# oraclefina/MSPI

Hardware: AMD Instinct MI355X
Metric: clips_per_sec (higher is better)
Workload: dtype f32 storage/accumulate; GEMMs as f16x3 split products on the f16 MFMA pipe; 1 GPU; x3dl motion encoder + ConvNeXt-T + ResNet18 audio + SyncBlock + decoder (AudioVisualSaliencyModel forward), batch 8/GPU, clips 3x16x224x224, spectrogram 1x257x300, inputs resident in HBM; global_batch=8, launch=hipGraph replay (mspi_amd.runtime.GraphPipeline), 2 batches in flight, stream_layout=2, parallelism=single GPU

## Files before the change

### include/mspi_hip.h

```cpp
#ifndef MSPI_HIP_H
#define MSPI_HIP_H

#include <stddef.h>
#include <stdint.h>

#ifdef __cplusplus
extern "C" {
#endif

#define MSPI_ABI_VERSION 2

typedef void* mspi_stream_t;

enum {
  MSPI_OK = 0,
  MSPI_EINVAL = -1,
  MSPI_ELAUNCH = -2,
  MSPI_ENODEV = -3
};

enum { MSPI_ACT_NONE = 0, MSPI_ACT_RELU = 1, MSPI_ACT_GELU = 2, MSPI_ACT_SIGMOID = 3, MSPI_ACT_SWISH = 4 };

enum { MSPI_PREC_F32 = 0, MSPI_PREC_F16X3 = 1 };

// ... 18 lines not shown
  int32_t prec;
  float w_scale;
  int32_t tile;
  const void* w_blocked;
} MspiConvDesc;

int mspi_conv_fwd(const MspiConvDesc* d, const float* x, const float* w, const float* bias ,
                  const float* res , const float* gate ,
                  float* y, mspi_stream_t stream);

size_t mspi_conv_splitk_ws_bytes(const MspiConvDesc* d, int32_t ksplit);
int mspi_conv_splitk_fwd(const MspiConvDesc* d, const float* x, const float* w, const float* bias, const float* res,
                         float* y, void* workspace, int32_t ksplit, mspi_stream_t stream);
int mspi_conv_variant(const MspiConvDesc* d, const float* x, const float* gate, int32_t ksplit);

int mspi_conv_last_config(void);

typedef struct MspiDwConvDesc {
  int32_t N, T, H, W, C;
  int64_t ldx, ldy;
  int32_t kT, kH, kW;
  int32_t strT, strH, strW;
  int32_t padT, padH, padW;
  int32_t To, Ho, Wo;
  int32_t act;
} MspiDwConvDesc;

int mspi_dwconv_fwd(const MspiDwConvDesc* d, const float* x, const float* w, const float* bias,
                    float* y, float* pool , mspi_stream_t stream);
int mspi_dwconv_pool_rows(const MspiDwConvDesc* d);
// ... 50 lines not shown
  float wa_scale;
} MspiX3dAbDesc;

int mspi_x3d_ab_supported(const MspiX3dAbDesc* d);
int mspi_x3d_ab_pool_rows(const MspiX3dAbDesc* d);
size_t mspi_x3d_ab_packed_bytes(int32_t Cin, int32_t Cmid);
int mspi_x3d_ab_fwd(const MspiX3dAbDesc* d, const void* x, const void* wa_packed, const void* bias_a, const void* wb,
                    const void* bias_b, void* u, void* pool , mspi_stream_t stream);
int mspi_x3d_ab_variant(const MspiX3dAbDesc* d);

int mspi_maxpool_fwd(const MspiDwConvDesc* d, const float* x, float* y, mspi_stream_t stream);

int mspi_upsample_fwd(const float* src, int64_t lds, float* dst, int64_t ldd, int32_t NT, int32_t H,
                      int32_t W, int32_t C, int32_t factor, int32_t accumulate, int32_t act,
                      mspi_stream_t stream);

int mspi_space_to_depth(const float* x, int64_t ldx, float* y, int64_t ldy, int32_t NT, int32_t H, int32_t W,
                        int32_t C, mspi_stream_t stream);

int mspi_rowgate(float* x, int64_t ldx, const float* mask, int64_t M, int32_t C, mspi_stream_t stream);

int mspi_logsumexp_sub(float* x, int32_t N, int32_t L, mspi_stream_t stream);

int mspi_mean_rows(const float* x, int64_t ldx, int64_t rows_per_sample_stride, float* out, int32_t N,
                   int32_t R, int32_t C, mspi_stream_t stream);

int mspi_mean_rows_slices(int32_t R);
int mspi_mean_rows_ws(const float* x, int64_t ldx, int64_t rows_per_sample_stride, float* out, float* ws, int32_t N,
                      int32_t R, int32_t C, mspi_stream_t stream);

// ... 113 lines not shown
```

### mspi_amd/_lib.py

```python
import ctypes as C
import os

_HERE = os.path.dirname(os.path.abspath(__file__))
LIB_PATH = os.environ.get("MSPI_LIB_PATH") or os.path.join(_HERE, "csrc", "libmspi_hip.so")

ACT_NONE, ACT_RELU, ACT_GELU, ACT_SIGMOID, ACT_SWISH = range(5)
PREC_F32, PREC_F16X3 = 0, 1


class MspiError(RuntimeError):
    pass


class ConvDesc(C.Structure):
    _fields_ = [
        ("N", C.c_int32), ("T", C.c_int32), ("H", C.c_int32), ("W", C.c_int32), ("C", C.c_int32),
        ("sN", C.c_int64), ("sT", C.c_int64), ("sH", C.c_int64), ("sW", C.c_int64), ("sC", C.c_int64),
        ("kT", C.c_int32), ("kH", C.c_int32), ("kW", C.c_int32),
        ("strT", C.c_int32), ("strH", C.c_int32), ("strW", C.c_int32),
        ("padT", C.c_int32), ("padH", C.c_int32), ("padW", C.c_int32),
        ("To", C.c_int32), ("Ho", C.c_int32), ("Wo", C.c_int32),
        ("Cout", C.c_int32),
        ("ldy", C.c_int64), ("ldw", C.c_int64), ("ldr", C.c_int64),
        ("act", C.c_int32),
# ... 74 lines not shown
class PermuteDesc(C.Structure):
    _fields_ = [("dims", C.c_int32 * 6), ("strides", C.c_int64 * 6), ("src_elems", C.c_int64)]


_P = C.c_void_p
_SIGNATURES = {
    "mspi_version": (C.c_int, []),
    "mspi_last_error": (C.c_char_p, []),
    "mspi_device_count": (C.c_int, []),
    "mspi_set_status_word": (C.c_int, [_P]),
    "mspi_conv_last_config": (C.c_int, []),
    "mspi_conv_splitk_ws_bytes": (C.c_size_t, [C.POINTER(ConvDesc), C.c_int32]),
    "mspi_conv_splitk_fwd": (C.c_int, [C.POINTER(ConvDesc), _P, _P, _P, _P, _P, _P, C.c_int32, _P]),
    "mspi_conv_fwd": (C.c_int, [C.POINTER(ConvDesc), _P, _P, _P, _P, _P, _P, _P]),
    "mspi_conv_variant": (C.c_int, [C.POINTER(ConvDesc), _P, _P, C.c_int32]),
    "mspi_dwconv_fwd": (C.c_int, [C.POINTER(DwConvDesc), _P, _P, _P, _P, _P, _P]),
    "mspi_dwconv_pool_rows": (C.c_int, [C.POINTER(DwConvDesc)]),
    "mspi_dwconv_variant": (C.c_int, [C.POINTER(DwConvDesc)]),
    "mspi_se_gate": (C.c_int, [_P, C.c_int32, C.c_float, _P, _P, _P, _P, _P, C.c_int32, C.c_int32, C.c_int32, _P]),
    "mspi_se_gate_variant": (C.c_int, [C.c_int32, C.c_int32]),
    "mspi_layernorm_variant": (C.c_int, [C.c_int32, C.c_int32]),
    "mspi_layernorm_fwd": (C.c_int, [_P, C.c_int64, C.c_int64, _P, C.c_int64, C.c_int64, _P, _P, C.c_float, C.c_int32,
                                      C.c_int32, C.c_int32, C.c_int32, _P, _P]),
    "mspi_attn_fwd": (C.c_int, [C.POINTER(AttnDesc), _P, _P, _P, _P, _P, _P, _P, _P, _P]),
    "mspi_attn_ws_bytes": (C.c_size_t, [C.POINTER(AttnDesc)]),
    "mspi_attn_fwd_ws": (C.c_int, [C.POINTER(AttnDesc), _P, _P, _P, _P, _P, _P, _P, _P, _P, _P]),
    "mspi_attn_variant": (C.c_int, [C.POINTER(AttnDesc), C.c_int32, C.c_int32, C.c_int32, C.c_int32]),
    "mspi_space_to_depth": (C.c_int, [_P, C.c_int64, _P, C.c_int64, C.c_int32, C.c_int32, C.c_int32, C.c_int32, _P]),
    "mspi_mvit_qk_augment": (C.c_int, [C.POINTER(MvitAugDesc), _P, _P, _P, _P, _P, _P, _P, _P]),
    "mspi_mvit_qk_augment_p": (C.c_int, [C.POINTER(MvitAugDesc), _P, _P, _P, C.c_int64, _P, _P, _P, _P, _P, _P]),
    "mspi_maxpool_fwd": (C.c_int, [C.POINTER(DwConvDesc), _P, _P, _P]),
    "mspi_upsample_fwd": (C.c_int, [_P, C.c_int64, _P, C.c_int64, C.c_int32, C.c_int32, C.c_int32, C.c_int32,
                                     C.c_int32, C.c_int32, C.c_int32, _P]),
    "mspi_rowgate": (C.c_int, [_P, C.c_int64, _P, C.c_int64, C.c_int32, _P]),
    "mspi_logsumexp_sub": (C.c_int, [_P, C.c_int32, C.c_int32, _P]),
    "mspi_mean_rows": (C.c_int, [_P, C.c_int64, C.c_int64, _P, C.c_int32, C.c_int32, C.c_int32, _P]),
    "mspi_mean_rows_slices": (C.c_int, [C.c_int32]),
    "mspi_mean_rows_ws": (C.c_int, [_P, C.c_int64, C.c_int64, _P, _P, C.c_int32, C.c_int32, C.c_int32, _P]),
    "mspi_neg_cosine": (C.c_int, [_P, _P, _P, C.c_int32, C.c_int32, C.c_float, C.c_int32, _P]),
    "mspi_add": (C.c_int, [_P, _P, _P, C.c_int64, _P]),
    "mspi_permute_fwd": (C.c_int, [C.POINTER(PermuteDesc), _P, _P, _P]),
    "mspi_permute_variant": (C.c_int, [C.POINTER(PermuteDesc), _P, _P]),
    "mspi_gated_sum_fwd": (C.c_int, [_P, _P, _P, _P, _P, C.c_int32, C.c_int64, C.c_int32, C.c_int32, _P]),
    "mspi_logspec_fwd": (C.c_int, [_P, C.c_int64, _P, _P, C.c_int32, _P, _P, C.c_int32, _P]),
    "mspi_resize_norm_fwd": (C.c_int, [_P, C.c_int32, C.c_int32, _P, _P, C.c_int64, C.c_int32, C.c_int32, _P, _P, C.c_int32,
                                        _P, _P, C.c_int32, _P, _P, _P]),
    "mspi_clip_resize_plan": (C.c_int, [_P, C.c_int32, C.c_int32, C.c_int32, C.c_int32, C.c_int32, _P]),
    "mspi_clip_resize_norm_fwd": (C.c_int, [_P, C.c_int32, C.c_int32, C.c_int32, _P, _P, _P, C.c_int32, C.c_int32, C.c_int64,
# ... 65 lines not shown
```

### mspi_amd/csrc/rowops.hip

```cpp
#include "common.h"

namespace mspi {

constexpr int LN_MAXC = 3072;

template <int LPR, int VPT>
__global__ __launch_bounds__(256) void layernorm_kernel(const float* __restrict__ x, long ldx, long sNx,
                                                        float* __restrict__ y, long ldy, long sNy,
                                                        const float* __restrict__ gamma,
                                                        const float* __restrict__ beta, float eps, long M, int R, int C,
                                                        int act, const float* __restrict__ table,
                                                        _Float16* __restrict__ ys, long ldys, long yplane) {
  constexpr int RPW = 64 / LPR;
  const int lane = threadIdx.x & 63;
  const int sub = lane % LPR;
  const long row = ((long)blockIdx.x * 4 + (threadIdx.x >> 6)) * RPW + lane / LPR;
  const bool rok = row < M;
  const long rr = rok ? row : 0;
  const long n = (long)((unsigned)rr / (unsigned)R);
  const int r = (int)(rr - n * R);
  const int nv = C >> 2;
  const float* xr = x + n * sNx + (long)r * ldx;
  float4 v[VPT];
  float s = 0.f;
// ... 187 lines not shown
    if (accumulate) {
      const float4 p = *reinterpret_cast<const float4*>(d);
      o.x += p.x; o.y += p.y; o.z += p.z; o.w += p.w;
    }
    if (act != MSPI_ACT_NONE) {
      auto fin = [&](auto act_c) {
        constexpr int ACT = decltype(act_c)::value;
        o.x = act_apply(o.x, ACT); o.y = act_apply(o.y, ACT); o.z = act_apply(o.z, ACT); o.w = act_apply(o.w, ACT);
      };
      MSPI_DISPATCH_ACT(act, fin)
    }
    *reinterpret_cast<float4*>(d) = o;
  }
}

__global__ __launch_bounds__(256) void s2d_kernel(const float* __restrict__ x, long ldx, float* __restrict__ y, long ldy,
                                                  int NT, int H, int W, int CV) {
  const int Ho = H / 2, Wo = W / 2;
  const long total = (long)NT * Ho * Wo * 4 * CV;
  for (long idx = (long)blockIdx.x * 256 + threadIdx.x; idx < total; idx += (long)gridDim.x * 256) {
    const int cv = (int)(idx % CV);
    long r = idx / CV;
    const int qd = (int)(r & 3);
    r >>= 2;
    const int wo = (int)(r % Wo);
    r /= Wo;
    const int ho = (int)(r % Ho);
    const long nt = r / Ho;
    const int dh = qd & 1, dw = qd >> 1;
    const float4 v = *reinterpret_cast<const float4*>(x + ((nt * H + 2 * ho + dh) * W + 2 * wo + dw) * ldx + cv * 4);
// ... 224 lines not shown

extern "C" int mspi_upsample_fwd(const float* src, int64_t lds, float* dst, int64_t ldd, int32_t NT, int32_t H,
                                 int32_t W, int32_t C, int32_t factor, int32_t accumulate, int32_t act,
                                 mspi_stream_t stream) {
  MSPI_REQUIRE(src && dst, "mspi_upsample_fwd: null argument");
  MSPI_REQUIRE(NT > 0 && H > 0 && W > 0 && C > 0 && factor >= 1, "mspi_upsample_fwd: bad extent");
  MSPI_REQUIRE((C & 3) == 0 && (lds & 3) == 0 && (ldd & 3) == 0 && lds >= C && ldd >= C && aligned16(src) && aligned16(dst),
               "mspi_upsample_fwd: C/ld must be multiples of 4, pointers 16-B aligned");
  const long total = (long)NT * H * factor * W * factor * (C / 4);
  MSPI_REQUIRE(total < (1L << 31), "mspi_upsample_fwd: more than 2^31 output vectors");
  hipLaunchKernelGGL(upsample_kernel, dim3(grid_for(total)), dim3(256), 0, (hipStream_t)stream, src, (long)lds, dst,
                     (long)ldd, NT, H, W, C / 4, factor, accumulate, act);
  return check_launch("mspi_upsample_fwd");
}

extern "C" int mspi_space_to_depth(const float* x, int64_t ldx, float* y, int64_t ldy, int32_t NT, int32_t H, int32_t W,
                                   int32_t C, mspi_stream_t stream) {
  MSPI_REQUIRE(x && y && NT > 0 && H > 0 && W > 0 && C > 0, "mspi_space_to_depth: bad argument");
  MSPI_REQUIRE((H & 1) == 0 && (W & 1) == 0, "mspi_space_to_depth: H and W must be even (PatchMerging pads odd sizes; not supported)");
  MSPI_REQUIRE((C & 3) == 0 && (ldx & 3) == 0 && (ldy & 3) == 0 && ldx >= C && ldy >= 4 * C && aligned16(x) && aligned16(y),
               "mspi_space_to_depth: C/ld multiples of 4, 16-B alignment");
  hipLaunchKernelGGL(s2d_kernel, dim3(grid_for((long)NT * H * W * (C / 4))), dim3(256), 0, (hipStream_t)stream, x, (long)ldx, y,
                     (long)ldy, NT, H, W, C / 4);
  return check_launch("mspi_space_to_depth");
}

extern "C" int mspi_rowgate(float* x, int64_t ldx, const float* mask, int64_t M, int32_t C, mspi_stream_t stream) {
  MSPI_REQUIRE(x && mask && M > 0 && C > 0, "mspi_rowgate: bad argument");
  MSPI_REQUIRE((C & 3) == 0 && (ldx & 3) == 0 && ldx >= C && aligned16(x), "mspi_rowgate: C/ldx must be multiples of 4");
  hipLaunchKernelGGL(rowgate_kernel, dim3(grid_for(M * (C / 4))), dim3(256), 0, (hipStream_t)stream, x, (long)ldx, mask,
// ... 47 lines not shown
```

### mspi_amd/engine.py

```python
import ctypes as C
import math

import torch

from . import _lib
from ._lib import (ACT_GELU, ACT_NONE, ACT_RELU, ACT_SIGMOID, ACT_SWISH, PREC_F16X3, PREC_F32, AttnDesc, ConvDesc,
                   DwConvDesc, MspiError, MvitAugDesc, check)

import os as _os
DEFAULT_PREC = {"f32": PREC_F32, "f16x3": PREC_F16X3}[_os.environ.get("MSPI_GEMM_PREC", "f16x3")]

__all__ = ["CL", "SP", "alloc", "alloc_sp", "pack_conv", "pack_dwconv", "PackedConv", "PackedDw", "conv", "dwconv", "maxpool",
           "layernorm", "attention", "upsample", "rowgate", "logsumexp_sub", "mean_rows", "neg_cosine",
           "se_gate", "add", "fold_bn", "ACT_NONE", "ACT_RELU", "ACT_GELU", "ACT_SIGMOID", "ACT_SWISH"]


def rup4(c):
    return (c + 3) // 4 * 4


AUTOTUNE = {"on": _os.environ.get("MSPI_AUTOTUNE", "0") == "1", "cache": {}, "reps": 3}


def autotune(on=True):
    AUTOTUNE["on"] = bool(on)


def save_autotune(path):
# ... 1 lines not shown
    with open(path, "w") as f:
        json.dump({repr(k): v for k, v in AUTOTUNE["cache"].items()}, f, indent=0, sort_keys=True)


def load_autotune(path):
    import ast
    import json
    with open(path) as f:
        AUTOTUNE["cache"].update({ast.literal_eval(k): int(v) for k, v in json.load(f).items()})
    return len(AUTOTUNE["cache"])


THIN = 100
SPLITK = 200
SPLITK_ENABLED = _os.environ.get("MSPI_SPLITK", "1") != "0"
THIN_DEFAULT = True
THIN_ENABLED = _os.environ.get("MSPI_THIN", "1") != "0"


_TUNE_LOG = _os.environ.get("MSPI_TUNE_LOG") == "1"


def _tune_conv(launch, key, candidates):
    best, best_t, times = -1, float("inf"), []
    e0, e1 = torch.cuda.Event(enable_timing=True), torch.cuda.Event(enable_timing=True)
    for tile in candidates:
        if launch(tile) != 0:
            continue
        e0.record()
        for _ in range(AUTOTUNE["reps"]):
# ... 630 lines not shown
    taps = pk.k[0] * pk.k[1] * pk.k[2]
    tm = _Timed("conv_gemm", 2.0 * M * taps * pk.cin * pk.cout,
                4.0 * (N * T * H * W * pk.cin + M * pk.cout * (2 if res is not None else 1) + pk.cout * taps * pk.cin),
                "M=%d K=%d(%dx%d) N=%d s=%s%s%s" % (M, taps * pk.cin, taps, pk.cin, pk.cout, pk.stride,
                                                  " +res" if res is not None else "", " +gate" if gate is not None else ""))
    args = (xptr, pk.w.data_ptr(), pk.bias.data_ptr() if pk.bias is not None else None,
            res.ptr if res is not None else None, gate.data_ptr() if gate is not None else None, out.ptr, _stream())
    rg = None
    if THIN_ENABLED and pk.thin is not None and isinstance(x, CL) and x.dense:
        rg = _lib.RowGemmDesc()
        rg.M, rg.K, rg.N = M, pk.cin_s, pk.cout_s
        rg.ldx, rg.ldy, rg.ldr, rg.ldg = x.ld, out.ld, d.ldr, pk.cin_s
        rg.act, rg.rows_per_sample, rg.w_scale = d.act, To * Ho * Wo, pk.w_scale
        rg_args = (xptr, pk.thin.data_ptr(), args[2], args[3], args[4], out.ptr, args[6])

    def launch(t):
        if t == THIN:
            return lib.mspi_rowgemm_fwd(C.byref(rg), *rg_args)
        if t >= SPLITK:
            S = t - SPLITK
            ws = torch.empty(S * M * pk.cout_s, dtype=torch.float32, device=dev)
            d.tile = 3
            return lib.mspi_conv_splitk_fwd(C.byref(d), args[0], args[1], args[2], args[3], args[5], ws.data_ptr(), S, args[6])
        d.tile = t
        return lib.mspi_conv_fwd(C.byref(d), *args)

    choice = -1
    key = (M, taps * pk.cin_s, pk.cout_s, pk.k, pk.stride, pk.prec, d.sC == 1, res is not None, gate is not None, rg is not None)
    if tile is not None:
        choice = tile
    elif AUTOTUNE["on"] and not torch.cuda.is_current_stream_capturing():
        choice = AUTOTUNE["cache"].get(key)
        if choice is None:
            cands = [1, 2, 3, 4]
            if pk.prec == PREC_F16X3 and d.sC == 1 and Cin % 4 == 0:
                cands += [6, 7, 9, 10] + ([8] if pk.cout_s <= 256 else [])
                if M >= 16384:
                    cands += [12, 13, 14]
            if rg is not None:
                cands.append(THIN)
            nk = pk.ldw // 32
            if SPLITK_ENABLED and gate is None and -(-M // 64) * -(-pk.cout_s // 64) <= 384 and nk >= 32:
                cands += [SPLITK + S for S in (2, 4, 8) if nk >= 8 * S]
            choice = _tune_conv(launch, key, cands)
    elif key in AUTOTUNE["cache"]:
        choice = AUTOTUNE["cache"][key]
    elif rg is not None and THIN_DEFAULT:
        choice = THIN
    if choice == THIN and rg is None:
        raise MspiError("conv: the thin-GEMM kernel does not cover this call")
    with tm:
        check(launch(choice), "mspi_rowgemm_fwd" if choice == THIN else "mspi_conv_splitk_fwd" if choice >= SPLITK else "mspi_conv_fwd")
        if Profiler.active is not None:
            if choice == THIN:
                tm.name = "rowgemm<%d,f16x3>" % rowgemm_ksb(pk.cin_s)
            elif choice >= SPLITK:
                tm.name = "conv_gemm<64,64,splitk%d>" % (choice - SPLITK)
            else:
                c = lib.mspi_conv_last_config()
                tm.name = "conv_gemm<%d,%d,%s,%s>" % (c >> 16, (c >> 4) & 0xFFF,
                                                      "dma" if c & 4 else ("s" if c & 1 else "v4") + ("w8" if c & 8 else ""),
                                                      "f16x3" if (c >> 1) & 1 else "f32")
    return out


def _dw_desc(x, k, s, p, out_ld):
    d = DwConvDesc()
    assert x.dense
    d.N, d.T, d.H, d.W, d.C = x.N, x.T, x.H, x.W, x.Cs
    d.ldx, d.ldy = x.ld, out_ld
# ... 263 lines not shown

def upsample(src, factor, dst=None, accumulate=False, act=ACT_NONE):
    lib = _lib.load()
    assert src.dense
    if dst is None:
        assert not accumulate
        dst = alloc(src.N, src.T, src.H * factor, src.W * factor, src.C, src.buf.device)
    assert (dst.N, dst.T, dst.H, dst.W) == (src.N, src.T, src.H * factor, src.W * factor) and dst.C == src.C
    assert dst.dense
    with _Timed("upsample", 0.0, 4.0 * (src.M + dst.M * (2 if accumulate else 1)) * src.C):
        check(lib.mspi_upsample_fwd(src.ptr, src.ld, dst.ptr, dst.ld, src.N * src.T, src.H, src.W, src.Cs, factor,
                                    1 if accumulate else 0, act, _stream()), "mspi_upsample_fwd")
    return dst


def rowgate(x, mask):
    lib = _lib.load()
    assert mask.M == x.M and mask.ld == 1
    assert x.dense and mask.dense
    with _Timed("rowgate", 0.0, 8.0 * x.M * x.C):
        check(lib.mspi_rowgate(x.ptr, x.ld, mask.ptr, x.M, x.Cs, _stream()), "mspi_rowgate")
    return x


def logsumexp_sub(t, N, L):
    lib = _lib.load()
    check(lib.mspi_logsumexp_sub(t.data_ptr(), N, L, _stream()), "mspi_logsumexp_sub")
    return t


# ... 84 lines not shown
```

### mspi_amd/model/model_utils.py

```python
import os

import numpy as np
import torch
import torch.nn as nn

from .. import engine as E
from .._lib import MspiError
from ..backbones.convnext import ConvNeXtTinyFeatures
from ..backbones.resnet import get_resnet18
from ..module import HipModule, to_cl
from .get_video_backbones import video_motion_extractor


def get_sinusoid_encoding_table(n_position, d_hid):
    pos = np.arange(n_position, dtype=np.float64).reshape(-1, 1)
    hid = np.arange(d_hid).reshape(1, -1)
    ang = pos / np.power(10000, 2 * (hid // 2) / d_hid)
    ang[:, 0::2] = np.sin(ang[:, 0::2])
    ang[:, 1::2] = np.cos(ang[:, 1::2])
    return torch.tensor(ang, dtype=torch.float, requires_grad=False).unsqueeze(0)


def _f(t):
    return t.detach().float().contiguous()
# ... 288 lines not shown
        s = self.side[i]
        if self.ENABLED and s in self.used:
            ev = torch.cuda.Event()
            ev.record(s)
            self.main.wait_event(ev)
            self.used.remove(s)

    def __exit__(self, *exc):
        for s in list(self.used):
            ev = torch.cuda.Event()
            ev.record(s)
            self.main.wait_event(ev)
        self.used = []
        self.kept = []
        return False


def _compose_lateral(c0, c1):
    w0 = c0.weight.detach().double().flatten(1)
    w1 = c1.weight.detach().double()[:, :, :, 0, 0]
    w = torch.einsum("omt,mi->oit", w1, w0)[:, :, :, None, None]
    b = torch.einsum("omt,m->o", w1, c0.bias.detach().double())
    return w.float(), b.float()


class _SaliencyBase(HipModule):

    def _build_decoder(self, cfg, vis_embed_dims, extra_c4, de_embed_dim=192):
        d = de_embed_dim
        for k in range(4):
# ... 35 lines not shown
        else:
            w, b, stride = seq[0].weight.detach().float(), seq[0].bias.detach().float(), (1, 1, 1)
        if split is None:
            return (E.pack_conv(w, b, None, stride, (0, 0, 0)),)
        return (E.pack_conv(w[:, :split].contiguous(), b, None, stride, (0, 0, 0)),
                E.pack_conv(w[:, split:].contiguous(), None, None, stride, (0, 0, 0)))

    def _pack_decoder(self, split=None):
        r = self.readout
        sa_w, sa_b = zip(*[E.fold_bn(m.conv_mask[0].conv.weight, None, m.conv_mask[0].bn) for m in (self.sa_0, self.sa_1, self.sa_2)])
        sa_cat = E.pack_conv(torch.cat(sa_w, 0), torch.cat(sa_b, 0), None, (1, 1, 1), (1, 1, 1), E.ACT_RELU)
        return {
            "sa_cat": sa_cat,
            "lat": [self._pack_lateral(k, split if k == 3 else None) for k in range(4)],
            "r0": E.pack_conv(r[0].weight, r[0].bias),
            "r1": E.pack_conv(r[1].weight, r[1].bias, r[2], (1, 1, 1), (1, 1, 1), E.ACT_RELU),
            "r4": E.pack_conv(r[4].weight, r[4].bias, r[5], (1, 1, 1), (0, 1, 1), E.ACT_RELU),
            "r8": E.pack_conv(r[8].weight, r[8].bias, None, (4, 1, 1), (0, 0, 0), E.ACT_NONE),
            "r10": E.pack_conv(r[10].weight, r[10].bias, None, (1, 1, 1), (0, 1, 1), E.ACT_RELU),
            "r12": E.pack_conv(r[12].weight, r[12].bias, None, (1, 1, 1), (0, 1, 1), E.ACT_NONE),
        }

    def _lateral(self, pk, k, xs, out=None):
        y = E.conv(xs[0], pk["lat"][k][0])
        if len(xs) == 2:
            y = E.conv(xs[1], pk["lat"][k][1], res=y)
        return getattr(self, "latlayer_%d" % k)[-1].run(y, out=out)

    def _laterals_012(self, pk, v1, v2, v3):
        B = v1.N
        cat = E.alloc(B, max(1, v1.T // (self.cfg.MODEL.LATERAL_STRIDE[0] if self.cfg.MODEL.LATERAL_BOOL[0] else 1)),
                      v1.H, v1.W, 4 * 192, v1.buf.device)
        s0 = self._lateral(pk, 0, [v1], out=cat.slice(0, 192))
        return cat, s0, self._lateral(pk, 1, [v2]), self._lateral(pk, 2, [v3])

    @torch.no_grad()
    def encode_frames(self, frames):
        self._check_eval()
        o1, o0 = self.image_encoder.run(frames.float()[:, :, None])
        return (o1.buf.view(o1.N, o1.H, o1.W, o1.ld)[..., :o1.C], o0.buf.view(o0.N, o0.H, o0.W, o0.ld)[..., :o0.C])

    @staticmethod
    def _wrap_frame_feats(frame_feats):
        outs = []
        for f in frame_feats:
            f = f.float().contiguous()
            n, h, w, c = f.shape
            outs.append(E.CL(f.view(-1), 0, n, 1, h, w, c, c))
        return outs

    def _premask(self, pk, masks):
        return E.conv(masks, pk["sa_cat"])

    def _fuse_readout(self, pk, cat, s0, s1, s2, s3, masks, pm):
        B = s0.N
        self.sa_2.run(s2, masks, pm.slice(64, 32))
        E.upsample(s3, 2, dst=s2, accumulate=True)
        self.sa_1.run(s1, masks, pm.slice(32, 32))
        E.upsample(s2, 2, dst=s1, accumulate=True)
        E.upsample(s3, 4, dst=s1, accumulate=True)
        self.sa_0.run(s0, masks, pm.slice(0, 32))
        E.upsample(s1, 2, dst=s0, accumulate=True)
        E.upsample(s2, 4, dst=s0, accumulate=True)
        E.upsample(s3, 8, dst=s0, accumulate=True)
        E.upsample(s1, 2, dst=cat.slice(192, 192))
        E.upsample(s2, 4, dst=cat.slice(384, 192))
        E.upsample(s3, 8, dst=cat.slice(576, 192))
        y = E.conv(E.conv(E.conv(cat, pk["r0"]), pk["r1"]), pk["r4"])
        y = E.upsample(E.conv(y, pk["r8"]), 4, act=E.ACT_RELU)
        y = E.conv(E.conv(y, pk["r10"]), pk["r12"])
        E.logsumexp_sub(y.buf, B, y.H * y.W)
        return y.buf.view(B, y.H, y.W)

    def _try_load(self, module_loader, path, what):
        if os.path.exists(path):
            module_loader(path)
        else:
            print("[mspi_amd] %s not found at %s: keeping random initialisation" % (what, path))

    def _pack_clips(self, clips):
        name = self.cfg.MODEL.MOTION_ENCODER
        if name == "slowfast4x16":
            return [torch.stack([clips[:, :, 0], clips[:, :, 4], clips[:, :, 12], clips[:, :, -1]], dim=2), clips]
# ... 142 lines not shown
```

Baseline: 651.5 clips/s.

## Add halo-staged 3x3 conv kernel and algebraically fuse decoder upsample-concat-conv

Result: faster. 672.3 clips/s, median of 6 (+3.2%).

```diff
diff --git a/include/mspi_hip.h b/include/mspi_hip.h
--- a/include/mspi_hip.h
+++ b/include/mspi_hip.h
@@ -56,6 +56,11 @@
                          float* y, void* workspace, int32_t ksplit, mspi_stream_t stream);
 int mspi_conv_variant(const MspiConvDesc* d, const float* x, const float* gate, int32_t ksplit);
 
+int mspi_conv_halo_fwd(const MspiConvDesc* d, const float* x, const float* bias, const float* res, const float* gate ,
+                       float* y, mspi_stream_t stream);
+int mspi_conv_halo_supported(const MspiConvDesc* d);
+int mspi_conv_halo_variant(const MspiConvDesc* d, const void* x);
+
 int mspi_conv_last_config(void);
 
 typedef struct MspiDwConvDesc {
@@ -136,6 +141,10 @@
 int mspi_upsample_fwd(const float* src, int64_t lds, float* dst, int64_t ldd, int32_t NT, int32_t H,
                       int32_t W, int32_t C, int32_t factor, int32_t accumulate, int32_t act,
                       mspi_stream_t stream);
+
+int mspi_upsample_sum_fwd(const float* const* srcs, const int64_t* lds, const int32_t* factors, int32_t J, float* dst,
+                          int64_t ldd, int32_t NT, int32_t Ho, int32_t Wo, int32_t C, int32_t accumulate, int32_t act,
+                          mspi_stream_t stream);
 
 int mspi_space_to_depth(const float* x, int64_t ldx, float* y, int64_t ldy, int32_t NT, int32_t H, int32_t W,
                         int32_t C, mspi_stream_t stream);
diff --git a/mspi_amd/_lib.py b/mspi_amd/_lib.py
--- a/mspi_amd/_lib.py
+++ b/mspi_amd/_lib.py
@@ -112,6 +112,9 @@
     "mspi_conv_splitk_fwd": (C.c_int, [C.POINTER(ConvDesc), _P, _P, _P, _P, _P, _P, C.c_int32, _P]),
     "mspi_conv_fwd": (C.c_int, [C.POINTER(ConvDesc), _P, _P, _P, _P, _P, _P, _P]),
     "mspi_conv_variant": (C.c_int, [C.POINTER(ConvDesc), _P, _P, C.c_int32]),
+    "mspi_conv_halo_fwd": (C.c_int, [C.POINTER(ConvDesc), _P, _P, _P, _P, _P, _P]),
+    "mspi_conv_halo_supported": (C.c_int, [C.POINTER(ConvDesc)]),
+    "mspi_conv_halo_variant": (C.c_int, [C.POINTER(ConvDesc), _P]),
     "mspi_dwconv_fwd": (C.c_int, [C.POINTER(DwConvDesc), _P, _P, _P, _P, _P, _P]),
     "mspi_dwconv_pool_rows": (C.c_int, [C.POINTER(DwConvDesc)]),
     "mspi_dwconv_variant": (C.c_int, [C.POINTER(DwConvDesc)]),
@@ -130,6 +133,8 @@
     "mspi_maxpool_fwd": (C.c_int, [C.POINTER(DwConvDesc), _P, _P, _P]),
     "mspi_upsample_fwd": (C.c_int, [_P, C.c_int64, _P, C.c_int64, C.c_int32, C.c_int32, C.c_int32, C.c_int32,
                                      C.c_int32, C.c_int32, C.c_int32, _P]),
+    "mspi_upsample_sum_fwd": (C.c_int, [_P, _P, _P, C.c_int32, _P, C.c_int64, C.c_int32, C.c_int32, C.c_int32, C.c_int32,
+                                         C.c_int32, C.c_int32, _P]),
     "mspi_rowgate": (C.c_int, [_P, C.c_int64, _P, C.c_int64, C.c_int32, _P]),
     "mspi_logsumexp_sub": (C.c_int, [_P, C.c_int32, C.c_int32, _P]),
     "mspi_mean_rows": (C.c_int, [_P, C.c_int64, C.c_int64, _P, C.c_int32, C.c_int32, C.c_int32, _P]),
diff --git a/mspi_amd/csrc/conv_halo.hip b/mspi_amd/csrc/conv_halo.hip
--- /dev/null
+++ b/mspi_amd/csrc/conv_halo.hip
@@ -0,0 +1,263 @@
+#include "conv_common.h"
+
+namespace mspi {
+
+__device__ __attribute__((aligned(16))) float g_halo_zero16[4] = {0.f, 0.f, 0.f, 0.f};
+
+typedef __attribute__((address_space(3))) void halo_lds_void;
+
+constexpr int HB_T = 4, HB_H = 8, HB_W = 8;
+constexpr int HH = HB_H + 2, HW = HB_W + 2;
+
+struct HaloArgs {
+  const float* x;
+  const _Float16* wb;
+  const float* bias;
+  const float* res;
+  float* y;
+  int N, T, H, W, C, Cout;
+  long sN, sT, sH, sW;
+  long ldy, ldw, ldr, wplane;
+  int nbt, nbh, nbw, tiles_n;
+  int act;
+  float out_scale;
+  int* status;
+};
+
+template <int KT, int TN>
+__global__ __launch_bounds__(512) void conv_halo_kernel(const HaloArgs p) {
+  constexpr int BN = 32 * TN;
+  constexpr int HT = HB_T + KT - 1;
+  constexpr int NCELL = HT * HH * HW;
+  constexpr int IMG_PLANE = NCELL * 64;
+  constexpr int P_BYTES = BN * 64;
+  constexpr int WSTAGE = 2 * P_BYTES;
+  constexpr int NGRP = BN / 16;
+  constexpr int HBI = (NGRP + 7) / 8;
+  constexpr int NLD = (NCELL * 8 + 511) / 512;
+  constexpr int NTAP = KT * 9;
+  __shared__ __attribute__((aligned(16))) unsigned char smem[2 * IMG_PLANE + 2 * WSTAGE];
+  unsigned char* wsm = smem + 2 * IMG_PLANE;
+
+  const int tid = threadIdx.x, lane = tid & 63, wave = tid >> 6;
+  const int li = lane & 31, lh = lane >> 5;
+  int b = blockIdx.x;
+  const int tile_n = b % p.tiles_n; b /= p.tiles_n;
+  const int bw_i = b % p.nbw; b /= p.nbw;
+  const int bh_i = b % p.nbh; b /= p.nbh;
+  const int bt_i = b % p.nbt;
+  const int n = b / p.nbt;
+  const int t0 = bt_i * HB_T, h0 = bh_i * HB_H, w0 = bw_i * HB_W, n0 = tile_n * BN;
+  const float* xn = p.x + (long)n * p.sN;
+
+  int g_off[NLD];
+#pragma unroll
+  for (int i = 0; i < NLD; ++i) {
+    const int e = tid + 512 * i;
+    const int cell = e >> 3, q = e & 7;
+    const int tt = cell / (HH * HW), rem = cell - tt * (HH * HW);
+    const int hh = rem / HW, ww = rem - hh * HW;
+    const int t = t0 - KT / 2 + tt, h = h0 - 1 + hh, w = w0 - 1 + ww;
+    const bool ok = cell < NCELL && (unsigned)t < (unsigned)p.T && (unsigned)h < (unsigned)p.H && (unsigned)w < (unsigned)p.W;
+    g_off[i] = ok ? (int)((long)t * p.sT + (long)h * p.sH + (long)w * p.sW) + q * 4 : -1;
+  }
+  float4 pre[NLD];
+  auto image_load = [&](int chunk) {
+#pragma unroll
+    for (int i = 0; i < NLD; ++i) {
+      const float* src = g_off[i] >= 0 ? xn + g_off[i] + chunk * 32 : g_halo_zero16;
+      pre[i] = *reinterpret_cast<const float4*>(src);
+    }
+  };
+  auto image_store = [&]() {
+#pragma unroll
+    for (int i = 0; i < NLD; ++i) {
+      const int e = tid + 512 * i;
+      const int cell = e >> 3, q = e & 7;
+      if (cell < NCELL) {
+        const float a4[4] = {pre[i].x, pre[i].y, pre[i].z, pre[i].w};
+        v4h h4, l4;
+#pragma unroll
+        for (int c = 0; c < 4; ++c) { _Float16 hh_, ll_; split_f16(a4[c], hh_, ll_); h4[c] = hh_; l4[c] = ll_; }
+        const int o = cell * 64 + ((((q >> 1) ^ (cell >> 2)) & 3) << 4) + (q & 1) * 8;
+        *reinterpret_cast<v4h*>(smem + o) = h4;
+        *reinterpret_cast<v4h*>(smem + IMG_PLANE + o) = l4;
+      }
+    }
+  };
+
+  const int b_seg = (lane & 3) ^ ((lane >> 4) & 3);
+  const int kt32 = (int)(p.ldw >> 5);
+  auto weights_issue = [&](int st, int kb) {
+    unsigned char* base = wsm + st * WSTAGE;
+#pragma unroll
+    for (int i = 0; i < HBI; ++i) {
+      const int g = i * 8 + wave;
+      if (g < NGRP) {
+        const bool ok = n0 + g * 16 < p.Cout;
+        const _Float16* q = p.wb + ((long)((n0 >> 4) + (ok ? g : 0)) * kt32 + kb) * 512 + (lane >> 2) * 32 + b_seg * 8;
+        const void* s_hi = ok ? (const void*)q : (const void*)g_halo_zero16;
+        const void* s_lo = ok ? (const void*)(q + p.wplane) : (const void*)g_halo_zero16;
+        __builtin_amdgcn_global_load_lds(s_hi, (halo_lds_void*)(base + g * 1024), 16, 0, 0);
+        __builtin_amdgcn_global_load_lds(s_lo, (halo_lds_void*)(base + P_BYTES + g * 1024), 16, 0, 0);
+      }
+    }
+  };
+
+  v16f acc[TN];
+#pragma unroll
+  for (int j = 0; j < TN; ++j)
+#pragma unroll
+    for (int r = 0; r < 16; ++r) acc[j][r] = 0.f;
+
+  const int cell0 = (wave >> 1) * (HH * HW) + ((wave & 1) * 4 + (li >> 3)) * HW + (li & 7);
+
+  const int nchunk = p.C >> 5;
+  const int nsteps = nchunk * NTAP;
+  image_load(0);
+  weights_issue(0, 0);
+  image_store();
+  asm volatile("s_waitcnt vmcnt(0)" ::: "memory");
+  __syncthreads();
+  int it = 0;
+  for (int chunk = 0; chunk < nchunk; ++chunk) {
+    int dt = 0, dh = 0, dw = 0;
+    for (int tap = 0; tap < NTAP; ++tap, ++it) {
+      const int cur = it & 1;
+      if (it + 1 < nsteps) {
+        const bool last = tap + 1 == NTAP;
+        weights_issue(cur ^ 1, last ? chunk + 1 : (tap + 1) * nchunk + chunk);
+        if (last) image_load(chunk + 1);
+      }
+      const int cell = cell0 + dt * (HH * HW) + dh * HW + dw;
+      const unsigned char* wbase = wsm + cur * WSTAGE;
+      const _Float16* Bh = reinterpret_cast<const _Float16*>(wbase);
+      const _Float16* Bl = reinterpret_cast<const _Float16*>(wbase + P_BYTES);
+#pragma unroll
+      for (int sub = 0; sub < 2; ++sub) {
+        const int oa = cell * 64 + ((((2 * lh + sub) ^ (cell >> 2)) & 3) << 4);
+        const v8h ah = *reinterpret_cast<const v8h*>(smem + oa);
+        const v8h al = *reinterpret_cast<const v8h*>(smem + IMG_PLANE + oa);
+#pragma unroll
+        for (int j = 0; j < TN; ++j) {
+          const int r = j * 32 + li;
+          const int o = r * 32 + (((2 * lh + sub) ^ ((r >> 2) & 3)) << 3);
+          const v8h bh = *reinterpret_cast<const v8h*>(&Bh[o]);
+          const v8h bl = *reinterpret_cast<const v8h*>(&Bl[o]);
+          if (!kSingleProduct) {
+            acc[j] = __builtin_amdgcn_mfma_f32_32x32x16_f16(al, bh, acc[j], 0, 0, 0);
+            acc[j] = __builtin_amdgcn_mfma_f32_32x32x16_f16(ah, bl, acc[j], 0, 0, 0);
+          }
+          acc[j] = __builtin_amdgcn_mfma_f32_32x32x16_f16(ah, bh, acc[j], 0, 0, 0);
+        }
+      }
+      if (++dw == 3) { dw = 0; if (++dh == 3) { dh = 0; ++dt; } }
+      asm volatile("s_waitcnt vmcnt(0)" ::: "memory");
+      __syncthreads();
+    }
+    if (chunk + 1 < nchunk) {
+      image_store();
+      __syncthreads();
+    }
+  }
+
+  const int t = t0 + (wave >> 1);
+  bool bad = false;
+  auto epilogue = [&](auto act_c) {
+    constexpr int ACT = decltype(act_c)::value;
+#pragma unroll
+    for (int j = 0; j < TN; ++j) {
+      const int col = n0 + j * 32 + li;
+      if (col >= p.Cout || t >= p.T) continue;
+      const float bv = p.bias ? p.bias[col] : 0.f;
+#pragma unroll
+      for (int r = 0; r < 16; ++r) {
+        const int h = h0 + (wave & 1) * 4 + (r >> 2), w = w0 + 4 * lh + (r & 3);
+        if (h < p.H && w < p.W) {
+          const long row = (((long)n * p.T + t) * p.H + h) * p.W + w;
+          const float pre_v = acc[j][r] * p.out_scale + bv + (p.res ? p.res[row * p.ldr + col] : 0.f);
+          bad |= nonfinite(pre_v);
+          p.y[row * p.ldy + col] = act_apply(pre_v, ACT);
+        }
+      }
+    }
+  };
+  MSPI_DISPATCH_ACT(p.act, epilogue)
+  report_nonfinite(p.status, bad);
+}
+
+template <int KT, int TN>
+static void launch_halo(const HaloArgs& a, unsigned grid, hipStream_t s) {
+  hipLaunchKernelGGL((conv_halo_kernel<KT, TN>), dim3(grid), dim3(512), 0, s, a);
+}
+
+}
+
+using namespace mspi;
+
+static int halo_select(const MspiConvDesc* d, const void* x) {
+  MSPI_REQUIRE(d && x, "mspi_conv_halo_fwd: null argument");
+  MSPI_REQUIRE(d->N > 0 && d->T > 0 && d->H > 0 && d->W > 0 && d->C > 0 && d->Cout > 0, "mspi_conv_halo_fwd: empty extent");
+  MSPI_REQUIRE((d->kT == 1 || d->kT == 3) && d->kH == 3 && d->kW == 3, "mspi_conv_halo_fwd: kernel (%d,%d,%d) is not (1|3,3,3)", d->kT,
+               d->kH, d->kW);
+  MSPI_REQUIRE(d->strT == 1 && d->strH == 1 && d->strW == 1, "mspi_conv_halo_fwd: stride (%d,%d,%d) is not 1", d->strT, d->strH, d->strW);
+  MSPI_REQUIRE(d->padT == d->kT / 2 && d->padH == 1 && d->padW == 1, "mspi_conv_halo_fwd: pad (%d,%d,%d) is not (kT/2,1,1)", d->padT,
+               d->padH, d->padW);
+  MSPI_REQUIRE(d->To == d->T && d->Ho == d->H && d->Wo == d->W, "mspi_conv_halo_fwd: output extent (%d,%d,%d) does not match the input's",
+               d->To, d->Ho, d->Wo);
+  MSPI_REQUIRE(d->prec == PREC_F16X3 && d->w_scale > 0.f, "mspi_conv_halo_fwd: f16x3 only (prec %d)", d->prec);
+  MSPI_REQUIRE(d->C % 32 == 0, "mspi_conv_halo_fwd: C = %d is not a multiple of 32", d->C);
+  MSPI_REQUIRE(d->sC == 1, "mspi_conv_halo_fwd: channels-last input only (sC = %ld)", (long)d->sC);
+  MSPI_REQUIRE(aligned16(x) && (d->sN & 3) == 0 && (d->sT & 3) == 0 && (d->sH & 3) == 0 && (d->sW & 3) == 0,
+               "mspi_conv_halo_fwd: input pointer and strides must be 16-B aligned");
+  MSPI_REQUIRE(d->sW >= d->C && d->sH > 0 && d->sT > 0 && d->sN > 0, "mspi_conv_halo_fwd: bad strides");
+  MSPI_REQUIRE((long)(d->T - 1) * d->sT + (long)(d->H - 1) * d->sH + (long)(d->W - 1) * d->sW + d->C < (1L << 31),
+               "mspi_conv_halo_fwd: sample too large for 32-bit offsets");
+  MSPI_REQUIRE(d->ldw == (long)d->kT * 9 * d->C, "mspi_conv_halo_fwd: ldw %ld != K", (long)d->ldw);
+  MSPI_REQUIRE(d->w_blocked && aligned16(d->w_blocked), "mspi_conv_halo_fwd: needs the blocked weight planes (w_blocked)");
+  MSPI_REQUIRE(d->ldy >= d->Cout, "mspi_conv_halo_fwd: ldy < Cout");
+  const int bn = d->Cout <= 64 ? 64 : d->Cout <= 128 ? 128 : 192;
+  const long grid = (long)d->N * ((d->T + HB_T - 1) / HB_T) * ((d->H + HB_H - 1) / HB_H) * ((d->W + HB_W - 1) / HB_W) * ((d->Cout + bn - 1) / bn);
+  MSPI_REQUIRE(grid < (1L << 31) && (long)d->N * d->T * d->H * d->W < (1L << 31), "mspi_conv_halo_fwd: problem too large");
+  return d->kT * 1000 + bn;
+}
+
+extern "C" int mspi_conv_halo_supported(const MspiConvDesc* d) {
+  static const float probe[4] __attribute__((aligned(16))) = {0.f, 0.f, 0.f, 0.f};
+  return d && halo_select(d, probe) > 0 ? 1 : 0;
+}
+
+extern "C" int mspi_conv_halo_variant(const MspiConvDesc* d, const void* x) { return halo_select(d, x); }
+
+extern "C" int mspi_conv_halo_fwd(const MspiConvDesc* d, const float* x, const float* bias, const float* res, const float* gate,
+                                  float* y, mspi_stream_t stream) {
+  MSPI_REQUIRE(d && x && y, "mspi_conv_halo_fwd: null argument");
+  MSPI_REQUIRE(!gate, "mspi_conv_halo_fwd: no gate");
+  const int variant = halo_select(d, x);
+  if (variant < 0) return variant;
+  MSPI_REQUIRE(!res || d->ldr >= d->Cout, "mspi_conv_halo_fwd: ldr < Cout");
+  const int bn = variant % 1000;
+  HaloArgs a;
+  a.x = x; a.wb = (const _Float16*)d->w_blocked; a.bias = bias; a.res = res; a.y = y;
+  a.N = d->N; a.T = d->T; a.H = d->H; a.W = d->W; a.C = d->C; a.Cout = d->Cout;
+  a.sN = d->sN; a.sT = d->sT; a.sH = d->sH; a.sW = d->sW;
+  a.ldy = d->ldy; a.ldw = d->ldw; a.ldr = d->ldr;
+  a.wplane = (long)((d->Cout + 15) / 16 * 16) * d->ldw;
+  a.nbt = (d->T + HB_T - 1) / HB_T; a.nbh = (d->H + HB_H - 1) / HB_H; a.nbw = (d->W + HB_W - 1) / HB_W;
+  a.tiles_n = (d->Cout + bn - 1) / bn;
+  a.act = d->act;
+  a.out_scale = 1.0f / d->w_scale;
+  a.status = g_status_word;
+  const unsigned grid = (unsigned)((long)d->N * a.nbt * a.nbh * a.nbw * a.tiles_n);
+  hipStream_t s = (hipStream_t)stream;
+  switch (variant) {
+    case 1064: launch_halo<1, 2>(a, grid, s); break;
+    case 1128: launch_halo<1, 4>(a, grid, s); break;
+    case 1192: launch_halo<1, 6>(a, grid, s); break;
+    case 3064: launch_halo<3, 2>(a, grid, s); break;
+    case 3128: launch_halo<3, 4>(a, grid, s); break;
+    case 3192: launch_halo<3, 6>(a, grid, s); break;
+    default: MSPI_REQUIRE(false, "mspi_conv_halo_fwd: variant %d is not instantiated", variant);
+  }
+  return check_launch("mspi_conv_halo_fwd");
+}
diff --git a/mspi_amd/csrc/rowops.hip b/mspi_amd/csrc/rowops.hip
--- a/mspi_amd/csrc/rowops.hip
+++ b/mspi_amd/csrc/rowops.hip
@@ -225,6 +225,76 @@
   }
 }
 
+struct UpSumSrc {
+  const float* p;
+  long ld;
+  int H, W, k;
+};
+struct UpSumArgs {
+  UpSumSrc s[3];
+};
+
+__device__ __forceinline__ float4 upsample_tap(const UpSumSrc& s, float inv, long nt, int ho, int wo, int cv) {
+  const int H = s.H, W = s.W;
+  const long lds = s.ld;
+  float fh = ((float)ho + 0.5f) * inv - 0.5f;
+  float fw = ((float)wo + 0.5f) * inv - 0.5f;
+  fh = fh < 0.f ? 0.f : fh;
+  fw = fw < 0.f ? 0.f : fw;
+  const int h0 = (int)fh, w0 = (int)fw;
+  const int h1 = h0 + (h0 < H - 1 ? 1 : 0), w1 = w0 + (w0 < W - 1 ? 1 : 0);
+  const float lh = fh - (float)h0, lw = fw - (float)w0;
+  const float* b = s.p + (nt * H * W) * lds + cv * 4;
+  const float4 v00 = *reinterpret_cast<const float4*>(b + ((long)h0 * W + w0) * lds);
+  const float4 v01 = *reinterpret_cast<const float4*>(b + ((long)h0 * W + w1) * lds);
+  const float4 v10 = *reinterpret_cast<const float4*>(b + ((long)h1 * W + w0) * lds);
+  const float4 v11 = *reinterpret_cast<const float4*>(b + ((long)h1 * W + w1) * lds);
+  const float c00 = (1.f - lh) * (1.f - lw), c01 = (1.f - lh) * lw, c10 = lh * (1.f - lw), c11 = lh * lw;
+  float4 o;
+  o.x = c00 * v00.x + c01 * v01.x + c10 * v10.x + c11 * v11.x;
+  o.y = c00 * v00.y + c01 * v01.y + c10 * v10.y + c11 * v11.y;
+  o.z = c00 * v00.z + c01 * v01.z + c10 * v10.z + c11 * v11.z;
+  o.w = c00 * v00.w + c01 * v01.w + c10 * v10.w + c11 * v11.w;
+  return o;
+}
+
+template <int J>
+__global__ __launch_bounds__(256) void upsample_sum_kernel(UpSumArgs a, float* __restrict__ dst, long ldd, int NT, int Ho,
+                                                           int Wo, int CV, int accumulate, int act) {
+  const long total = (long)NT * Ho * Wo * CV;
+  float inv[J];
+#pragma unroll
+  for (int j = 0; j < J; ++j) inv[j] = 1.f / (float)a.s[j].k;
+  for (long idx = (long)blockIdx.x * 256 + threadIdx.x; idx < total; idx += (long)gridDim.x * 256) {
+    const unsigned ui = (unsigned)idx;
+    const int cv = (int)(ui % (unsigned)CV);
+    unsigned pos = ui / (unsigned)CV;
+    const int wo = (int)(pos % (unsigned)Wo);
+    pos /= (unsigned)Wo;
+    const int ho = (int)(pos % (unsigned)Ho);
+    const long nt = (long)(pos / (unsigned)Ho);
+    float* d = dst + ((nt * Ho + ho) * Wo + wo) * ldd + cv * 4;
+    float4 o = upsample_tap(a.s[0], inv[0], nt, ho, wo, cv);
+    if (accumulate) {
+      const float4 p = *reinterpret_cast<const float4*>(d);
+      o.x += p.x; o.y += p.y; o.z += p.z; o.w += p.w;
+    }
+#pragma unroll
+    for (int j = 1; j < J; ++j) {
+      const float4 u = upsample_tap(a.s[j], inv[j], nt, ho, wo, cv);
+      o.x += u.x; o.y += u.y; o.z += u.z; o.w += u.w;
+    }
+    if (act != MSPI_ACT_NONE) {
+      auto fin = [&](auto act_c) {
+        constexpr int ACT = decltype(act_c)::value;
+        o.x = act_apply(o.x, ACT); o.y = act_apply(o.y, ACT); o.z = act_apply(o.z, ACT); o.w = act_apply(o.w, ACT);
+      };
+      MSPI_DISPATCH_ACT(act, fin)
+    }
+    *reinterpret_cast<float4*>(d) = o;
+  }
+}
+
 __global__ __launch_bounds__(256) void s2d_kernel(const float* __restrict__ x, long ldx, float* __restrict__ y, long ldy,
                                                   int NT, int H, int W, int CV) {
   const int Ho = H / 2, Wo = W / 2;
@@ -479,6 +549,36 @@
   return check_launch("mspi_upsample_fwd");
 }
 
+extern "C" int mspi_upsample_sum_fwd(const float* const* srcs, const int64_t* lds, const int32_t* factors, int32_t J,
+                                     float* dst, int64_t ldd, int32_t NT, int32_t Ho, int32_t Wo, int32_t C,
+                                     int32_t accumulate, int32_t act, mspi_stream_t stream) {
+  MSPI_REQUIRE(srcs && lds && factors && dst, "mspi_upsample_sum_fwd: null argument");
+  MSPI_REQUIRE(J >= 1 && J <= 3, "mspi_upsample_sum_fwd: 1 to 3 sources");
+  MSPI_REQUIRE(NT > 0 && Ho > 0 && Wo > 0 && C > 0, "mspi_upsample_sum_fwd: bad extent");
+  MSPI_REQUIRE((C & 3) == 0 && (ldd & 3) == 0 && ldd >= C && aligned16(dst),
+               "mspi_upsample_sum_fwd: C/ld must be multiples of 4, pointers 16-B aligned");
+  UpSumArgs a = {};
+  for (int j = 0; j < J; ++j) {
+    const int k = factors[j];
+    MSPI_REQUIRE(k >= 1 && Ho % k == 0 && Wo % k == 0, "mspi_upsample_sum_fwd: every factor must be >= 1 and divide Ho and Wo");
+    MSPI_REQUIRE(srcs[j] && (lds[j] & 3) == 0 && lds[j] >= C && aligned16(srcs[j]),
+                 "mspi_upsample_sum_fwd: C/ld must be multiples of 4, pointers 16-B aligned");
+    a.s[j].p = srcs[j];
+    a.s[j].ld = (long)lds[j];
+    a.s[j].H = Ho / k;
+    a.s[j].W = Wo / k;
+    a.s[j].k = k;
+  }
+  const long total = (long)NT * Ho * Wo * (C / 4);
+  MSPI_REQUIRE(total < (1L << 31), "mspi_upsample_sum_fwd: more than 2^31 output vectors");
+  const dim3 grid(grid_for(total)), block(256);
+  hipStream_t st = (hipStream_t)stream;
+  if (J == 1) hipLaunchKernelGGL((upsample_sum_kernel<1>), grid, block, 0, st, a, dst, (long)ldd, NT, Ho, Wo, C / 4, accumulate, act);
+  else if (J == 2) hipLaunchKernelGGL((upsample_sum_kernel<2>), grid, block, 0, st, a, dst, (long)ldd, NT, Ho, Wo, C / 4, accumulate, act);
+  else hipLaunchKernelGGL((upsample_sum_kernel<3>), grid, block, 0, st, a, dst, (long)ldd, NT, Ho, Wo, C / 4, accumulate, act);
+  return check_launch("mspi_upsample_sum_fwd");
+}
+
 extern "C" int mspi_space_to_depth(const float* x, int64_t ldx, float* y, int64_t ldy, int32_t NT, int32_t H, int32_t W,
                                    int32_t C, mspi_stream_t stream) {
   MSPI_REQUIRE(x && y && NT > 0 && H > 0 && W > 0 && C > 0, "mspi_space_to_depth: bad argument");
diff --git a/mspi_amd/engine.py b/mspi_amd/engine.py
--- a/mspi_amd/engine.py
+++ b/mspi_amd/engine.py
@@ -11,7 +11,7 @@
 DEFAULT_PREC = {"f32": PREC_F32, "f16x3": PREC_F16X3}[_os.environ.get("MSPI_GEMM_PREC", "f16x3")]
 
 __all__ = ["CL", "SP", "alloc", "alloc_sp", "pack_conv", "pack_dwconv", "PackedConv", "PackedDw", "conv", "dwconv", "maxpool",
-           "layernorm", "attention", "upsample", "rowgate", "logsumexp_sub", "mean_rows", "neg_cosine",
+           "layernorm", "attention", "upsample", "upsample_sum", "rowgate", "logsumexp_sub", "mean_rows", "neg_cosine",
            "se_gate", "add", "fold_bn", "ACT_NONE", "ACT_RELU", "ACT_GELU", "ACT_SIGMOID", "ACT_SWISH"]
 
 
@@ -43,6 +43,8 @@
 THIN = 100
 SPLITK = 200
 SPLITK_ENABLED = _os.environ.get("MSPI_SPLITK", "1") != "0"
+HALO = 300
+HALO_ENABLED = _os.environ.get("MSPI_CONV_HALO", "1") != "0"
 THIN_DEFAULT = True
 THIN_ENABLED = _os.environ.get("MSPI_THIN", "1") != "0"
 
@@ -703,9 +705,14 @@
         rg.act, rg.rows_per_sample, rg.w_scale = d.act, To * Ho * Wo, pk.w_scale
         rg_args = (xptr, pk.thin.data_ptr(), args[2], args[3], args[4], out.ptr, args[6])
 
+    halo = bool(HALO_ENABLED and gate is None and d.w_blocked and pk.k[1:] == (3, 3) and xptr % 16 == 0 and
+                lib.mspi_conv_halo_supported(C.byref(d)))
+
     def launch(t):
         if t == THIN:
             return lib.mspi_rowgemm_fwd(C.byref(rg), *rg_args)
+        if t == HALO:
+            return lib.mspi_conv_halo_fwd(C.byref(d), args[0], args[2], args[3], None, out.ptr, args[6])
         if t >= SPLITK:
             S = t - SPLITK
             ws = torch.empty(S * M * pk.cout_s, dtype=torch.float32, device=dev)
@@ -715,7 +722,7 @@
         return lib.mspi_conv_fwd(C.byref(d), *args)
 
     choice = -1
-    key = (M, taps * pk.cin_s, pk.cout_s, pk.k, pk.stride, pk.prec, d.sC == 1, res is not None, gate is not None, rg is not None)
+    key = (M, taps * pk.cin_s, pk.cout_s, pk.k, pk.stride, pk.prec, d.sC == 1, res is not None, gate is not None, rg is not None, halo)
     if tile is not None:
         choice = tile
     elif AUTOTUNE["on"] and not torch.cuda.is_current_stream_capturing():
@@ -728,6 +735,8 @@
                     cands += [12, 13, 14]
             if rg is not None:
                 cands.append(THIN)
+            if halo:
+                cands.append(HALO)
             nk = pk.ldw // 32
             if SPLITK_ENABLED and gate is None and -(-M // 64) * -(-pk.cout_s // 64) <= 384 and nk >= 32:
                 cands += [SPLITK + S for S in (2, 4, 8) if nk >= 8 * S]
@@ -738,11 +747,17 @@
         choice = THIN
     if choice == THIN and rg is None:
         raise MspiError("conv: the thin-GEMM kernel does not cover this call")
+    if choice == HALO and not halo:
+        raise MspiError("conv: the halo-staged kernel does not cover this call")
     with tm:
-        check(launch(choice), "mspi_rowgemm_fwd" if choice == THIN else "mspi_conv_splitk_fwd" if choice >= SPLITK else "mspi_conv_fwd")
+        check(launch(choice), "mspi_rowgemm_fwd" if choice == THIN else "mspi_conv_halo_fwd" if choice == HALO else
+              "mspi_conv_splitk_fwd" if choice >= SPLITK else "mspi_conv_fwd")
         if Profiler.active is not None:
             if choice == THIN:
                 tm.name = "rowgemm<%d,f16x3>" % rowgemm_ksb(pk.cin_s)
+            elif choice == HALO:
+                v = lib.mspi_conv_halo_variant(C.byref(d), xptr)
+                tm.name = "conv_halo<%d,%d,f16x3>" % (v // 1000, v % 1000)
             elif choice >= SPLITK:
                 tm.name = "conv_gemm<64,64,splitk%d>" % (choice - SPLITK)
             else:
@@ -1036,6 +1051,22 @@
     return dst
 
 
+def upsample_sum(dst, srcs, accumulate=True, act=ACT_NONE):
+    lib = _lib.load()
+    J = len(srcs)
+    for s, k in srcs:
+        assert s.dense and s.C == dst.C and (dst.N, dst.T) == (s.N, s.T)
+        assert k >= 1 and (dst.H, dst.W) == (s.H * k, s.W * k)
+    assert dst.dense
+    ptrs = (C.c_void_p * max(J, 1))(*[s.ptr for s, _ in srcs])
+    lds = (C.c_int64 * max(J, 1))(*[s.ld for s, _ in srcs])
+    ks = (C.c_int32 * max(J, 1))(*[k for _, k in srcs])
+    with _Timed("upsample_sum", 0.0, 4.0 * (sum(s.M for s, _ in srcs) + dst.M * (2 if accumulate else 1)) * dst.C):
+        check(lib.mspi_upsample_sum_fwd(ptrs, lds, ks, J, dst.ptr, dst.ld, dst.N * dst.T, dst.H, dst.W, dst.Cs,
+                                        1 if accumulate else 0, act, _stream()), "mspi_upsample_sum_fwd")
+    return dst
+
+
 def rowgate(x, mask):
     lib = _lib.load()
     assert mask.M == x.M and mask.ld == 1
diff --git a/mspi_amd/model/model_utils.py b/mspi_amd/model/model_utils.py
--- a/mspi_amd/model/model_utils.py
+++ b/mspi_amd/model/model_utils.py
@@ -326,6 +326,9 @@
         self.used = []
         self.kept = []
         return False
+
+
+DECODER_FUSED = os.environ.get("MSPI_DECODER_FUSED", "1") != "0"
 
 
 def _compose_lateral(c0, c1):
@@ -391,6 +394,7 @@
             "sa_cat": sa_cat,
             "lat": [self._pack_lateral(k, split if k == 3 else None) for k in range(4)],
             "r0": E.pack_conv(r[0].weight, r[0].bias),
+            "r0_parts": self._pack_r0_parts(r[0]),
             "r1": E.pack_conv(r[1].weight, r[1].bias, r[2], (1, 1, 1), (1, 1, 1), E.ACT_RELU),
             "r4": E.pack_conv(r[4].weight, r[4].bias, r[5], (1, 1, 1), (0, 1, 1), E.ACT_RELU),
             "r8": E.pack_conv(r[8].weight, r[8].bias, None, (4, 1, 1), (0, 0, 0), E.ACT_NONE),
@@ -398,6 +402,16 @@
             "r12": E.pack_conv(r[12].weight, r[12].bias, None, (1, 1, 1), (0, 1, 1), E.ACT_NONE),
         }
 
+    @staticmethod
+    def _r0_parts(weight, bias):
+        w = weight.detach().float().flatten(1)
+        d = w.shape[1] // 4
+        w0 = w[:, :d]
+        return [(w0.contiguous(), bias.detach().float())] + [((w0 + w[:, j * d:(j + 1) * d]).contiguous(), None) for j in (1, 2, 3)]
+
+    def _pack_r0_parts(self, conv):
+        return [E.pack_conv(w, b) for w, b in self._r0_parts(conv.weight, conv.bias)]
+
     def _lateral(self, pk, k, xs, out=None):
         y = E.conv(xs[0], pk["lat"][k][0])
         if len(xs) == 2:
@@ -405,6 +419,8 @@
         return getattr(self, "latlayer_%d" % k)[-1].run(y, out=out)
 
     def _laterals_012(self, pk, v1, v2, v3):
+        if DECODER_FUSED:
+            return None, self._lateral(pk, 0, [v1]), self._lateral(pk, 1, [v2]), self._lateral(pk, 2, [v3])
         B = v1.N
         cat = E.alloc(B, max(1, v1.T // (self.cfg.MODEL.LATERAL_STRIDE[0] if self.cfg.MODEL.LATERAL_BOOL[0] else 1)),
                       v1.H, v1.W, 4 * 192, v1.buf.device)
@@ -434,16 +450,24 @@
         self.sa_2.run(s2, masks, pm.slice(64, 32))
         E.upsample(s3, 2, dst=s2, accumulate=True)
         self.sa_1.run(s1, masks, pm.slice(32, 32))
-        E.upsample(s2, 2, dst=s1, accumulate=True)
-        E.upsample(s3, 4, dst=s1, accumulate=True)
-        self.sa_0.run(s0, masks, pm.slice(0, 32))
-        E.upsample(s1, 2, dst=s0, accumulate=True)
-        E.upsample(s2, 4, dst=s0, accumulate=True)
-        E.upsample(s3, 8, dst=s0, accumulate=True)
-        E.upsample(s1, 2, dst=cat.slice(192, 192))
-        E.upsample(s2, 4, dst=cat.slice(384, 192))
-        E.upsample(s3, 8, dst=cat.slice(576, 192))
-        y = E.conv(E.conv(E.conv(cat, pk["r0"]), pk["r1"]), pk["r4"])
+        if cat is None:
+            E.upsample_sum(s1, [(s2, 2), (s3, 4)])
+            self.sa_0.run(s0, masks, pm.slice(0, 32))
+            p0, p1, p2, p3 = pk["r0_parts"]
+            y = E.conv(s0, p0)
+            E.upsample_sum(y, [(E.conv(s1, p1), 2), (E.conv(s2, p2), 4), (E.conv(s3, p3), 8)])
+        else:
+            E.upsample(s2, 2, dst=s1, accumulate=True)
+            E.upsample(s3, 4, dst=s1, accumulate=True)
+            self.sa_0.run(s0, masks, pm.slice(0, 32))
+            E.upsample(s1, 2, dst=s0, accumulate=True)
+            E.upsample(s2, 4, dst=s0, accumulate=True)
+            E.upsample(s3, 8, dst=s0, accumulate=True)
+            E.upsample(s1, 2, dst=cat.slice(192, 192))
+            E.upsample(s2, 4, dst=cat.slice(384, 192))
+            E.upsample(s3, 8, dst=cat.slice(576, 192))
+            y = E.conv(cat, pk["r0"])
+        y = E.conv(E.conv(y, pk["r1"]), pk["r4"])
         y = E.upsample(E.conv(y, pk["r8"]), 4, act=E.ACT_RELU)
         y = E.conv(E.conv(y, pk["r10"]), pk["r12"])
         E.logsumexp_sub(y.buf, B, y.H * y.W)
```
